# IuvenisSapiens/Qwen3-TTS-Rust

Measured on AMD Instinct MI355X. Metric: audio-seconds generated per second (aggregate over GPUs) = concurrent real-time streams; RTF and first-chunk latency from the single-utterance leg, higher is better.
Workload: dtype i8

## Files before the change

### include/q3tts.h

```cpp
#ifndef Q3TTS_H
#define Q3TTS_H
#include <stdint.h>
#include <stddef.h>
#include "q3tts_spec.h"
#ifdef __cplusplus
extern "C" {
#endif

#define Q3TTS_OK 0
#define Q3TTS_ERR -1

const char* q3tts_last_error(void);
int q3tts_version(void);
int q3tts_device_count(void);

typedef struct q3tts_sampler_config {
    float temperature;
    int32_t top_k;
    float top_p;
    int32_t has_seed;
    uint64_t seed;
} q3tts_sampler_config;
void q3tts_sampler_config_default(q3tts_sampler_config* c);

// ... 350 lines not shown
                     const int32_t* job_page0, const int32_t* job_n_pages, const int32_t* job_first, const int32_t* job_n_dst,
                     const int32_t* slots, int32_t n_slots, int32_t save);
int q3tts_op_feedback_rows(const q3tts_assets* a, const int32_t* codes, int32_t n, const int32_t* trail_ids, int32_t n_trail, float* rows);
enum { Q3TTS_GEMM_AUTO = 0, Q3TTS_GEMM_SKINNY4 = 1, Q3TTS_GEMM_SKINNY8 = 2, Q3TTS_GEMM_SKINNY16 = 3,
       Q3TTS_GEMM_F32_1 = 4, Q3TTS_GEMM_F32_2 = 5,
       Q3TTS_GEMM_H1 = 6, Q3TTS_GEMM_H1_EPL = 7, Q3TTS_GEMM_H2 = 8, Q3TTS_GEMM_H2_EPL = 9,
       Q3TTS_GEMM_H3 = 10, Q3TTS_GEMM_H3_EPL = 11 };
enum { Q3TTS_EPI_NONE = 0, Q3TTS_EPI_GELU = 1, Q3TTS_EPI_RES_SCALE = 2 , Q3TTS_EPI_RES = 3 ,
       Q3TTS_EPI_SNAKE = 4  };
typedef struct q3tts_codec_gemm_desc {
    int32_t M, N, cin, taps, dil;
    const float* A; int64_t a_rows; int32_t lda, a_segT, a_skip;
    int32_t a_split, o_split;
    const float* W; const float* bias;
    int32_t epi; const float* res; int64_t res_floats; int32_t ldr, r_segT; int64_t r_skip;
    const float* scale; const float* snake_ea; const float* snake_ib;
    float* out; int64_t out_floats, out_off; int32_t ldo, o_segT; int64_t o_skip;
    int64_t ws_floats;
    int32_t form, ksplit, reducer;
    int32_t form_ran, ksplit_ran, reducer_ran;
} q3tts_codec_gemm_desc;
int q3tts_op_codec_gemm(q3tts_codec_gemm_desc* d);
int q3tts_codec_gemm_plan(q3tts_codec_gemm_desc* d);

enum { Q3TTS_CK_RVQ_SUM = 0, Q3TTS_CK_RMSNORM_ROWS = 1, Q3TTS_CK_LAYERNORM_ROWS = 2, Q3TTS_CK_ROPE_APPEND = 3, Q3TTS_CK_WINDOW_ATTN = 4,
       Q3TTS_CK_SWIGLU_ROWS = 5, Q3TTS_CK_DWCONV7 = 6, Q3TTS_CK_SNAKE = 7, Q3TTS_CK_SNAKE_SPLIT = 8, Q3TTS_CK_CONV_OUT_WAVE = 9,
       Q3TTS_CK_CONV_OUT_WIN = 10, Q3TTS_CK_HIST_LOAD = 11, Q3TTS_CK_HIST_SAVE = 12, Q3TTS_CK_HIST_ZERO = 13 };
typedef struct q3tts_codec_kernel_desc {
    int32_t kernel;
    int32_t G, T, C, H;
    int32_t n_heads, head_dim, window; float rope_base, eps, bias;
    const int64_t* meta;
    const int64_t* codes; int32_t n_q, cb_size;
    int32_t n_streams, stream;
    const float* in[3]; int64_t in_floats[3];
    const float* p0; const float* p1; int64_t p0_floats, p1_floats;
    float* out[3]; int64_t out_floats[3];
} q3tts_codec_kernel_desc;
int q3tts_op_codec_kernel(q3tts_codec_kernel_desc* d);

enum { Q3TTS_ATTN_AUTO = 0, Q3TTS_ATTN_UNFUSED = 1 , Q3TTS_ATTN_FUSED = 2 ,
       Q3TTS_ATTN_SHORT1 = 3, Q3TTS_ATTN_SHORT2 = 4 , Q3TTS_ATTN_GGML = 5  };
typedef struct q3tts_attention_desc {
    int32_t n_head, n_kv, n_layer, layer, ntok;
    const float* qkv; int32_t qkv_stride;
    const float* q_norm; const float* k_norm;
// ... 121 lines not shown
```

### qwen3-tts-rust_amd/csrc/capi_ops.cpp

```cpp
#include "../../include/q3tts.h"
#include "transformer.h"
#include "host_logic.h"
#include "kdev.h"
#include "codec.h"
#include "kernels.h"
#include "pcm_out.h"
#include "tsm.h"
#include "mel.h"

using namespace q3;
#define Q3_API_BEGIN try {
#define Q3_API_END(failval) } catch (const std::exception& ex) { set_last_error(ex.what()); return failval; } catch (...) { set_last_error("unknown error"); return failval; }
static void require_gpu() {
    int n = 0;
    if (hipGetDeviceCount(&n) != hipSuccess || n <= 0) throw Error("no HIP device available: the HIP path is the only compute path (no CPU fallback)");
}

static int attention_op_plan(const q3tts_attention_desc& d) {
    AttnPlanIn a;
    a.ntok = d.ntok; a.fused = d.fused != 0; a.fused_max_tok = d.fused_max_tok; a.same_seq = d.same_seq != 0; a.short_attn_min = d.short_attn_min;
    a.n_head = d.n_head; a.n_kv = d.n_kv; a.hpw1_max = d.hpw1_max > 0 ? d.hpw1_max : short_attn_hpw1_max();
    a.float_mode = d.float_mode != 0; a.ggml_mode = d.ggml_mode != 0;
    return plan_attention(a);
}
// ... 859 lines not shown
        else launch_sample_pred(0, a, B);
        Q3_LAUNCH_CHECK();
    }
    Q3_HIP(hipDeviceSynchronize());
    dout.download((q3_u64*)d.out_raw, raw.size());
    ddraw.download(d.draws_out, B);
    for (int i = 0; i < nl; i++) for (int b = 0; b < B; b++) d.tokens[(size_t)i * B + b] = key_code(d.out_raw[(size_t)i * slots + (size_t)b * d.out_stride]);
    return Q3TTS_OK;
    Q3_API_END(Q3TTS_ERR)
}

int q3tts_op_codec_gemm(q3tts_codec_gemm_desc* d) {
    Q3_API_BEGIN
    require_gpu();
    codec_gemm_run(d);
    return Q3TTS_OK;
    Q3_API_END(Q3TTS_ERR)
}

int q3tts_codec_gemm_plan(q3tts_codec_gemm_desc* d) {
    Q3_API_BEGIN
    codec_gemm_plan_only(d);
    return Q3TTS_OK;
    Q3_API_END(Q3TTS_ERR)
}

int q3tts_op_codec_kernel(q3tts_codec_kernel_desc* d) {
    Q3_API_BEGIN
    require_gpu();
    codec_kernel_run(d);
    return Q3TTS_OK;
    Q3_API_END(Q3TTS_ERR)
}

int q3tts_op_project(const float* x, const float* w, const float* b, int32_t n_in, int32_t n_out, float* y) {
    Q3_API_BEGIN
    require_gpu();
    Q3_CHECK(x && w && b && y && n_in >= 1 && n_out >= 1, "bad arguments");
    const std::vector<float> wb = project_wblk(w, n_in, n_out);
    DevBuf<float> dx(n_in), dw(wb.size()), db(n_out), dy(n_out);
    dx.upload(x, n_in); dw.upload(wb.data(), wb.size()); db.upload(b, n_out);
    launch_project_blk(0, dx.p, n_in, dw.p, db.p, n_in, n_out, dy.p, n_out, 1);
    Q3_LAUNCH_CHECK();
    Q3_HIP(hipDeviceSynchronize());
    dy.download(y, n_out);
    return Q3TTS_OK;
// ... 593 lines not shown
```

### qwen3-tts-rust_amd/csrc/codec.h

```cpp
#pragma once
#include "q3_common.h"
#include <memory>
#include <string>
#include <vector>

struct q3tts_codec_gemm_desc;
struct q3tts_codec_kernel_desc;

namespace q3 {

struct CodecStateEntry { std::string name; int64_t offset; int rows, cols; };

class CodecDecoder {
public:
    std::vector<CodecStateEntry> state_layout() const;
    size_t state_floats() const;
    void state_export(int stream, float* out, size_t n_floats) const;
    void state_import(int stream, const float* in, size_t n_floats);
    CodecDecoder(const std::string& gguf_path, int n_streams, int max_frames_per_call, int n_lanes = 1, int max_group = 1);
    int max_group() const;
    int n_lanes() const;
    ~CodecDecoder();
    int samples_per_frame() const;
    void reset(int stream);
    void reset_async(hipStream_t st, int stream);
    int snapshot_async(hipStream_t st, int stream);
    void restore_async(hipStream_t st, int snapshot, int stream, const float* pcm_tail = nullptr);
    void snapshot_free(int snapshot);
    size_t snapshot_bytes() const;
    int snapshots_live() const;
    int decode(hipStream_t st, int stream, const int64_t* codes, int n_frames, bool is_last, float* pcm);
    int decode_async(hipStream_t st, int stream, const int64_t* codes, int n_frames, bool is_last, float* pcm_pinned, int lane = 0);
    int decode_group_async(hipStream_t st, int G, const int* streams, const int64_t* codes, int n_frames, float* const* pcm_pinned, int lane = 0,
                           const q3tts_pcm_format* fmt = nullptr, int64_t* n_out = nullptr, const int32_t* rate = nullptr);
    void tsm_flush_async(hipStream_t st, int stream, void* dst, int64_t* n_out, int lane = 0);
    void tsm_stats(int64_t* chunks, int64_t* frames_out, int64_t* flushes) const;
    void pcm_out_stats(int64_t* chunks_converted, int64_t* samples_out) const;
    double flops_per_frame() const;
private:
    struct Impl;
    std::unique_ptr<Impl> impl_;
};

void codec_gemm_run(q3tts_codec_gemm_desc* d);
void codec_gemm_plan_only(q3tts_codec_gemm_desc* d);
void codec_kernel_run(q3tts_codec_kernel_desc* d);

}
```

### qwen3-tts-rust_amd/csrc/codec.hip

```cpp
#include "codec.h"
#include "../../include/q3tts.h"
#include "gguf.h"
#include "kernels.h"
#include "pcm_out.h"
#include "tsm.h"
#include <atomic>
#include <cmath>
#include <cstdlib>
#include <map>

namespace q3 {

typedef float f32x16 __attribute__((ext_vector_type(16)));

enum { EPI_NONE = 0, EPI_GELU = 1, EPI_RES_SCALE = 2, EPI_RES = 3, EPI_SNAKE = 4 };

struct GemmArgs {
    const float* A; int lda;
    int cin, dil;
    const float* W;
    const float* wscale;
    const float* bias;
    float* out; int ldo;
    int M, N, K;
// ... 258 lines not shown
        for (int e = tid; e < BM * (BN / 4); e += 256) {
            const int rl = e / (BN / 4), cl = (e % (BN / 4)) * 4, row = m0 + rl, col = n0 + cl;
            if (row >= g.M || col >= g.N) continue;
            const float4 t4 = *reinterpret_cast<const float4*>(&Ct[rl][cl]);
            if (ksplit > 1) *reinterpret_cast<float4*>(g.ws + ((size_t)blockIdx.z * g.M + row) * g.N + col) = t4;
            else gemm_epilogue_store4(g, t4, row, col);
        }
    } else {
        const int col = n0 + wn * 32 + (lane & 31);
        if (col < g.N) {
#pragma unroll
            for (int t = 0; t < MR; t++)
#pragma unroll
                for (int r = 0; r < 16; r++) {
                    const int row = m0 + (wm * MR + t) * 32 + (r & 3) + 8 * (r >> 2) + 4 * (lane >> 5);
                    if (row < g.M) {
                        if (ksplit > 1) g.ws[((size_t)blockIdx.z * g.M + row) * g.N + col] = acc[t][r];
                        else gemm_store(g, row, col, gemm_epilogue(g, acc[t][r], row, col));
                    }
                }
        }
    }
}
template <int MR, int NT, int BK, int EPL, int PF, bool SPLIT>
__global__ void __launch_bounds__(256) k_conv_gemm_h3(GemmArgs g, const _Float16* __restrict__ Wh, const _Float16* __restrict__ Wl) {
    constexpr int BM = 128 * MR, BN = 32 * NT, LD = BK + 8;
    constexpr int KQ = BK / 4, KC = BK / 8;
    constexpr int NA = BM * KQ / 256;
    constexpr int NB = (BN * KC + 255) / 256;
    constexpr int CLD = BN + 4;
    struct Stage { _Float16 Ah[BM][LD], Al[BM][LD], Bh[BN][LD], Bl[BN][LD]; };
    union Shared { Stage s; float Ct[EPL ? BM : 1][CLD]; };
    __shared__ __attribute__((aligned(16))) Shared sh;
    auto& Ah = sh.s.Ah; auto& Al = sh.s.Al; auto& Bh = sh.s.Bh; auto& Bl = sh.s.Bl;
    const int tid = threadIdx.x, lane = tid & 63, wave = tid >> 6;
    int tile_m = blockIdx.y, tile_n = blockIdx.x;
    if (g.xcd_swizzle) {
        const int nwg = gridDim.x * gridDim.y, orig = blockIdx.y * gridDim.x + blockIdx.x;
        const int xcd = orig & 7, q8 = nwg >> 3, r8 = nwg & 7;
        const int wgid = (xcd < r8 ? xcd * (q8 + 1) : r8 * (q8 + 1) + (xcd - r8) * q8) + (orig >> 3);
        tile_n = wgid % gridDim.x; tile_m = wgid / gridDim.x;
    }
    const int m0 = tile_m * BM, n0 = tile_n * BN;
    const int ksplit = gridDim.z, kper = g.K / ksplit, kbeg = blockIdx.z * kper, kend = kbeg + kper;
    f32x16 acc[MR][NT];
#pragma unroll
    for (int t = 0; t < MR; t++)
#pragma unroll
        for (int u = 0; u < NT; u++)
#pragma unroll
            for (int i = 0; i < 16; i++) acc[t][u][i] = 0.0f;
    int arow[NA];
#pragma unroll
    for (int i = 0; i < NA; i++) { int mm = m0 + (tid + i * 256) / KQ; mm = mm < g.M ? mm : g.M - 1; arow[i] = mm + seg_of(mm, g.a_segT) * g.a_skip; }
    struct Regs { float4 ra[NA]; uint4 rh[NB], rl[NB]; };
    auto fetch = [&](Regs& s, int k0) {
        const int j = k0 / g.cin, ci0 = k0 % g.cin;
#pragma unroll
        for (int i = 0; i < NA; i++) {
            const int kq = (tid + i * 256) % KQ;
            const size_t row = (size_t)(arow[i] + j * g.dil);
            if constexpr (SPLIT) s.ra[i] = load_a4_split_raw(g, row, ci0 + 4 * kq);
            else s.ra[i] = *reinterpret_cast<const float4*>(g.A + row * g.lda + ci0 + 4 * kq);
        }
#pragma unroll
        for (int i = 0; i < NB; i++) {
            int e = tid + i * 256;
            e = e < BN * KC ? e : e - 256;
            const int r = e / KC, wk = 8 * (e % KC);
            s.rh[i] = *reinterpret_cast<const uint4*>(Wh + (size_t)(n0 + r) * g.K + k0 + wk);
            s.rl[i] = *reinterpret_cast<const uint4*>(Wl + (size_t)(n0 + r) * g.K + k0 + wk);
        }
    };
    auto stash = [&](const Regs& s) {
#pragma unroll
        for (int i = 0; i < NA; i++) {
            const int e = tid + i * 256, r = e / KQ, kq = e % KQ;
            if constexpr (SPLIT) {
                *reinterpret_cast<float2*>(&Ah[r][4 * kq]) = make_float2(s.ra[i].x, s.ra[i].y);
                *reinterpret_cast<float2*>(&Al[r][4 * kq]) = make_float2(s.ra[i].z, s.ra[i].w);
            } else {
                const float x[4] = {s.ra[i].x, s.ra[i].y, s.ra[i].z, s.ra[i].w};
                h4v hi, lo;
#pragma unroll
                for (int c = 0; c < 4; c++) { hi[c] = (_Float16)x[c]; lo[c] = (_Float16)(x[c] - (float)hi[c]); }
                *reinterpret_cast<h4v*>(&Ah[r][4 * kq]) = hi;
                *reinterpret_cast<h4v*>(&Al[r][4 * kq]) = lo;
            }
        }
#pragma unroll
        for (int i = 0; i < NB; i++) {
            const int e = tid + i * 256, r = e / KC, wk = 8 * (e % KC);
            if (e < BN * KC) { *reinterpret_cast<uint4*>(&Bh[r][wk]) = s.rh[i]; *reinterpret_cast<uint4*>(&Bl[r][wk]) = s.rl[i]; }
        }
    };
    auto multiply = [&]() {
#pragma unroll
        for (int kk = 0; kk < BK; kk += 16) {
            const int ko = kk + 8 * (lane >> 5);
            if constexpr (MR == 1) {
                const int ar = wave * 32 + (lane & 31);
                const h8v ah = *reinterpret_cast<const h8v*>(&Ah[ar][ko]);
                const h8v al = *reinterpret_cast<const h8v*>(&Al[ar][ko]);
#pragma unroll
                for (int u = 0; u < NT; u++) {
                    const h8v bh = *reinterpret_cast<const h8v*>(&Bh[u * 32 + (lane & 31)][ko]);
                    const h8v bl = *reinterpret_cast<const h8v*>(&Bl[u * 32 + (lane & 31)][ko]);
                    acc[0][u] = __builtin_amdgcn_mfma_f32_32x32x16_f16(al, bh, acc[0][u], 0, 0, 0);
                    acc[0][u] = __builtin_amdgcn_mfma_f32_32x32x16_f16(ah, bl, acc[0][u], 0, 0, 0);
                    acc[0][u] = __builtin_amdgcn_mfma_f32_32x32x16_f16(ah, bh, acc[0][u], 0, 0, 0);
                }
            } else {
                h8v bh[NT], bl[NT];
#pragma unroll
                for (int u = 0; u < NT; u++) {
                    bh[u] = *reinterpret_cast<const h8v*>(&Bh[u * 32 + (lane & 31)][ko]);
                    bl[u] = *reinterpret_cast<const h8v*>(&Bl[u * 32 + (lane & 31)][ko]);
                }
#pragma unroll
                for (int t = 0; t < MR; t++) {
                    const int ar = (wave * MR + t) * 32 + (lane & 31);
                    const h8v ah = *reinterpret_cast<const h8v*>(&Ah[ar][ko]);
                    const h8v al = *reinterpret_cast<const h8v*>(&Al[ar][ko]);
#pragma unroll
                    for (int u = 0; u < NT; u++) {
                        acc[t][u] = __builtin_amdgcn_mfma_f32_32x32x16_f16(al, bh[u], acc[t][u], 0, 0, 0);
                        acc[t][u] = __builtin_amdgcn_mfma_f32_32x32x16_f16(ah, bl[u], acc[t][u], 0, 0, 0);
                        acc[t][u] = __builtin_amdgcn_mfma_f32_32x32x16_f16(ah, bh[u], acc[t][u], 0, 0, 0);
                    }
                    __builtin_amdgcn_sched_barrier(0);
                }
            }
        }
    };
    auto lds_barrier = [] { asm volatile("s_waitcnt lgkmcnt(0)\n\ts_barrier" ::: "memory"); };
    float wsc[NT];
#pragma unroll
    for (int u = 0; u < NT; u++) wsc[u] = g.wscale[n0 + u * 32 + (lane & 31)];
    Regs st[PF];
#pragma unroll
    for (int j = 0; j < PF; j++)
        if (kbeg + j * BK < kend) fetch(st[j], kbeg + j * BK);
    int k0 = kbeg;
    for (; k0 + 2 * PF * BK <= kend; k0 += PF * BK) {
#pragma unroll
        for (int j = 0; j < PF; j++) {
            stash(st[j]);
            lds_barrier();
            fetch(st[j], k0 + (j + PF) * BK);
            multiply();
            lds_barrier();
        }
    }
    for (; k0 < kend; k0 += PF * BK) {
#pragma unroll
        for (int j = 0; j < PF; j++) {
            if (k0 + j * BK < kend) {
                stash(st[j]);
                lds_barrier();
                if (k0 + (j + PF) * BK < kend) fetch(st[j], k0 + (j + PF) * BK);
                multiply();
                lds_barrier();
            }
        }
    }
#pragma unroll
    for (int u = 0; u < NT; u++)
#pragma unroll
        for (int t = 0; t < MR; t++)
#pragma unroll
            for (int r = 0; r < 16; r++) acc[t][u][r] *= wsc[u];
    __syncthreads();
    auto epilogue_rows = [&](const f32x16 (&a)[NT], int row0) {
#pragma unroll
        for (int r = 0; r < 16; r++) {
            const int row = row0 + (r & 3) + 8 * (r >> 2) + 4 * (lane >> 5);
            if (row < g.M) {
#pragma unroll
                for (int u = 0; u < NT; u++) {
                    const int col = n0 + u * 32 + (lane & 31);
                    if (col < g.N) {
                        if (ksplit > 1) g.ws[((size_t)blockIdx.z * g.M + row) * g.N + col] = a[u][r];
                        else gemm_store(g, row, col, gemm_epilogue(g, a[u][r], row, col));
                    }
                }
// ... 141 lines not shown
    const bool skinny = f <= Q3TTS_GEMM_SKINNY16, f32 = f == Q3TTS_GEMM_F32_1 || f == Q3TTS_GEMM_F32_2, h3 = f >= Q3TTS_GEMM_H3;
    const bool epl = f == Q3TTS_GEMM_H1_EPL || f == Q3TTS_GEMM_H2_EPL || f == Q3TTS_GEMM_H3_EPL;
    const bool ws_a16 = (reinterpret_cast<uintptr_t>(g.ws) & 15) == 0;
    if (skinny) {
        if (g.M > (f == Q3TTS_GEMM_SKINNY4 ? 4 : f == Q3TTS_GEMM_SKINNY8 ? 8 : 16)) return "skinny form: M exceeds its row count";
        if (p.ks != 1) return "skinny form: no split-K";
        return nullptr;
    }
    if (f32 && (g.cin % 16 != 0 || (g.K / p.ks) % 16 != 0)) return "f32 form: cin and K / ksplit must be multiples of 16";
    if (!f32) {
        if (!has_split_w || !g.wscale) return "split-f16 form without split weights";
        if (g.cin % 32 != 0 || (g.K / p.ks) % 32 != 0) return "split-f16 form: cin and K / ksplit must be multiples of 32";
        if (h3 && g.N % 96 != 0) return "h3 form: N must be a multiple of 96";
        if (epl && !(epilogue4_ok(g) && ws_a16)) return "16-byte epilogue form: pointers / strides not 16-byte aligned or N % 4 != 0";
    }
    if (p.ks > 1) {
        if (p.ks > 64) return "ksplit too large";
        if ((size_t)p.ks * g.M * g.N > ws_floats) return "split-K workspace too small";
        if (p.red != 0 && p.red != 1) return "split-K needs a reducer (0 or 1)";
        if (p.red == 1 && !(epilogue4_ok(g) && ws_a16)) return "k_splitk_reduce4: pointers / strides not 16-byte aligned or N % 4 != 0";
    } else if (p.red != -1) return "a reducer without split-K";
    return nullptr;
}
static void launch_gemm(hipStream_t st, const GemmArgs& g, const GemmPlan& p, const _Float16* wh, const _Float16* wl) {
    const dim3 b256(256);
    const unsigned ks = (unsigned)p.ks;
#define Q3_H(MRV, EPLV, GRID) do { if (g.a_split) hipLaunchKernelGGL((k_conv_gemm_h<MRV, EPLV, true>), GRID, b256, 0, st, g, wh, wl); \
                                   else hipLaunchKernelGGL((k_conv_gemm_h<MRV, EPLV, false>), GRID, b256, 0, st, g, wh, wl); } while (0)
#define Q3_H3(EPLV, PFV) do { if (g.a_split) hipLaunchKernelGGL((k_conv_gemm_h3<1, 3, 32, EPLV, PFV, true>), grid3, b256, 0, st, g, wh, wl); \
                              else hipLaunchKernelGGL((k_conv_gemm_h3<1, 3, 32, EPLV, PFV, false>), grid3, b256, 0, st, g, wh, wl); } while (0)
    const dim3 grid_sk((g.N + 7) / 8), grid_t((g.N + 63) / 64, (g.M + 127) / 128, ks), grid_s((g.N + 63) / 64, (g.M + 63) / 64, ks);
    const dim3 grid3(g.N / 96, (g.M + 127) / 128, ks);
    switch (p.form) {
    case Q3TTS_GEMM_SKINNY4: hipLaunchKernelGGL((k_skinny_gemm<4>), grid_sk, dim3(512), 0, st, g); break;
    case Q3TTS_GEMM_SKINNY8: hipLaunchKernelGGL((k_skinny_gemm<8>), grid_sk, dim3(512), 0, st, g); break;
    case Q3TTS_GEMM_SKINNY16: hipLaunchKernelGGL((k_skinny_gemm<16>), grid_sk, dim3(512), 0, st, g); break;
    case Q3TTS_GEMM_F32_1: hipLaunchKernelGGL((k_conv_gemm<1>), dim3((g.N + 127) / 128, (g.M + 31) / 32, ks), b256, 0, st, g); break;
    case Q3TTS_GEMM_F32_2: hipLaunchKernelGGL((k_conv_gemm<2>), dim3((g.N + 63) / 64, (g.M + 63) / 64, ks), b256, 0, st, g); break;
    case Q3TTS_GEMM_H1: Q3_H(1, 0, grid_s); break;
    case Q3TTS_GEMM_H1_EPL: Q3_H(1, 1, grid_s); break;
    case Q3TTS_GEMM_H2: Q3_H(2, 0, grid_t); break;
    case Q3TTS_GEMM_H2_EPL: Q3_H(2, 1, grid_t); break;
    case Q3TTS_GEMM_H3: Q3_H3(0, 1); break;
    case Q3TTS_GEMM_H3_EPL: Q3_H3(1, 1); break;
    default: throw Error("unknown GEMM form");
    }
#undef Q3_H
#undef Q3_H3
    if (p.ks > 1) {
        const size_t n = (size_t)g.M * g.N;
        if (p.red == 1) hipLaunchKernelGGL(k_splitk_reduce4, dim3((unsigned)((n / 4 + 255) / 256)), b256, 0, st, g, p.ks);
        else hipLaunchKernelGGL(k_splitk_reduce, dim3((unsigned)((n + 255) / 256)), b256, 0, st, g, p.ks);
    }
}
static int xcd_swizzle_on() { static const int on = [] { const char* e = std::getenv("Q3_CODEC_XCD"); return e ? atoi(e) : 1; }(); return on; }
static void gemm(hipStream_t st, GemmArgs g, float* ws, size_t ws_floats, const _Float16* wh = nullptr, const _Float16* wl = nullptr) {
    g.ws = ws;
    g.xcd_swizzle = xcd_swizzle_on();
    launch_gemm(st, g, plan_gemm(g, ws_floats, wh != nullptr), wh, wl);
}

struct RowMap { int segT, skip, off; };
__device__ __forceinline__ size_t map_row(const RowMap& m, int r) { return (size_t)r + (size_t)(m.segT == SEG_NONE ? 0 : r / m.segT) * m.skip + m.off; }
static RowMap plain_map() { return RowMap{SEG_NONE, 0, 0}; }

__global__ void k_rvq_sum(const int64_t* __restrict__ codes, const float* const* __restrict__ cb, int n_q, int cb_size, int cb_dim,
                          float* __restrict__ out, int ldo, RowMap om) {
    const int t = blockIdx.y, d = blockIdx.x * 256 + threadIdx.x;
    if (d >= cb_dim) return;
    float acc = 0.0f;
    for (int q = 0; q < n_q; q++) {
// ... 930 lines not shown
static void check_desc(const q3tts_codec_gemm_desc& d) {
    Q3_CHECK(d.M >= 1 && d.N >= 1 && d.cin >= 1 && d.taps >= 1 && d.dil >= 1 && d.epi >= EPI_NONE && d.epi <= EPI_SNAKE, "bad codec GEMM descriptor");
    Q3_CHECK(d.a_segT >= 0 && d.o_segT >= 0 && d.r_segT >= 0 && d.a_skip >= 0 && d.o_skip >= 0 && d.r_skip >= 0 && d.out_off >= 0 && d.ws_floats >= 0,
             "negative segment / offset fields");
    Q3_CHECK(d.A && d.W && d.out && d.lda >= d.cin && d.ldo >= d.N, "codec GEMM: A, W and out are required; lda >= cin, ldo >= N");
    const long long m = d.M - 1;
    const long long arow = m + (d.a_segT > 0 ? m / d.a_segT * d.a_skip : 0) + (long long)(d.taps - 1) * d.dil;
    Q3_CHECK(arow < d.a_rows, "A rows read beyond a_rows");
    Q3_CHECK(d.out_off + m * d.ldo + (d.o_segT > 0 ? m / d.o_segT * d.o_skip : 0) + d.N <= d.out_floats, "output rows beyond out_floats");
    if (d.epi == EPI_RES || d.epi == EPI_RES_SCALE)
        Q3_CHECK(d.res && d.ldr >= d.N && m * d.ldr + (d.r_segT > 0 ? m / d.r_segT * d.r_skip : 0) + d.N <= d.res_floats, "residual rows beyond res_floats");
    Q3_CHECK(d.epi != EPI_RES_SCALE || d.scale, "EPI_RES_SCALE needs scale");
    Q3_CHECK(d.epi != EPI_SNAKE || (d.snake_ea && d.snake_ib), "EPI_SNAKE needs ea / ib");
}
void codec_gemm_plan_only(q3tts_codec_gemm_desc* d) {
    Q3_CHECK(d && d->M >= 1 && d->N >= 1 && d->cin >= 1 && d->taps >= 1 && d->out_off >= 0, "bad codec GEMM descriptor");
    GemmArgs g = desc_args(*d);
    auto at = [](const float* p, long long off) { return reinterpret_cast<float*>((p ? reinterpret_cast<uintptr_t>(p) : (uintptr_t)256) + 4 * (uintptr_t)off); };
    g.A = at(d->A, 0); g.W = at(d->W, 0); g.bias = d->bias; g.res = at(d->res, 0); g.scale = at(d->scale, 0);
    g.snake_ea = at(d->snake_ea, 0); g.snake_ib = at(d->snake_ib, 0); g.out = at(d->out, d->out_off); g.ws = at(nullptr, 0);
    const GemmPlan p = plan_gemm(g, (size_t)d->ws_floats, true);
    d->form_ran = p.form; d->ksplit_ran = p.ks; d->reducer_ran = p.red;
}
void codec_gemm_run(q3tts_codec_gemm_desc* d) {
    Q3_CHECK(d, "null codec GEMM descriptor");
    check_desc(*d);
    GemmArgs g = desc_args(*d);
    const int N = g.N, K = g.K;
    const bool res_used = g.epi == EPI_RES || g.epi == EPI_RES_SCALE;
    DevBuf<float> dA((size_t)d->a_rows * d->lda), dW((size_t)N * K), dsc(N), dbias(d->bias ? N : 0), dres(res_used ? d->res_floats : 0);
    DevBuf<float> dscale(d->scale ? N : 0), dea(d->snake_ea ? N : 0), dib(d->snake_ib ? N : 0), dout(d->out_floats), dws(std::max<int64_t>(d->ws_floats, 4));
    DevBuf<_Float16> dwh((size_t)N * K), dwl((size_t)N * K);
    g.A = dA.p; g.W = dW.p; g.wscale = dsc.p; g.bias = dbias.p; g.res = dres.p; g.scale = dscale.p; g.snake_ea = dea.p; g.snake_ib = dib.p;
    g.out = dout.p + d->out_off; g.ws = dws.p;
    const GemmPlan p = d->form == Q3TTS_GEMM_AUTO ? plan_gemm(g, (size_t)d->ws_floats, true) : GemmPlan{d->form, d->ksplit, d->reducer};
    if (const char* why = gemm_plan_error(g, p, (size_t)d->ws_floats, true)) throw Error(std::string("codec GEMM form not applicable: ") + why);
    std::vector<_Float16> h((size_t)N * K), l((size_t)N * K);
    std::vector<float> sc(N);
    split_weights(d->W, N, K, h.data(), l.data(), sc.data());
    dA.upload(d->A, dA.n); dW.upload(d->W, dW.n); dwh.upload(h.data(), h.size()); dwl.upload(l.data(), l.size()); dsc.upload(sc.data(), N);
    if (d->bias) dbias.upload(d->bias, N);
    if (res_used) dres.upload(d->res, dres.n);
    if (d->scale) dscale.upload(d->scale, N);
    if (d->snake_ea) dea.upload(d->snake_ea, N);
    if (d->snake_ib) dib.upload(d->snake_ib, N);
    dout.upload(d->out, dout.n);
// ... 112 lines not shown
```

### qwen3-tts-rust_amd/python/q3tts/__init__.py

```python
import ctypes as C
import os
import numpy as np

_HERE = os.path.dirname(os.path.abspath(__file__))
PKG_ROOT = os.path.dirname(os.path.dirname(_HERE))
LIB_PATH = os.path.join(PKG_ROOT, "libq3tts.so")
_lib = None


class Q3Error(RuntimeError):
    pass


class SamplerConfig(C.Structure):
    _fields_ = [("temperature", C.c_float), ("top_k", C.c_int32), ("top_p", C.c_float), ("has_seed", C.c_int32),
                ("seed", C.c_uint64)]


class GenOptions(C.Structure):
    _fields_ = [("repetition_penalty", C.c_float), ("predictor_temperature", C.c_float), ("predictor_top_k", C.c_int32),
                ("predictor_top_p", C.c_float)]


GEN_DEFAULTS = {"repetition_penalty": 1.0, "predictor_temperature": 0.0, "predictor_top_k": 0, "predictor_top_p": 1.0}
# ... 34 lines not shown
    "q3tts_engine_create", "q3tts_engine_destroy", "q3tts_generate_batch", "q3tts_engine_stats", "q3tts_engine_reset_stats",
    "q3tts_engine_set_instrument", "q3tts_engine_bytes_per_step", "q3tts_assets_open", "q3tts_assets_close", "q3tts_engine_assets",
    "q3tts_assets_codec_embedding", "q3tts_assets_text_embedding", "q3tts_assets_tts_pad", "q3tts_prompt_build_core",
    "q3tts_prompt_build_clone", "q3tts_sampler_new", "q3tts_sampler_free", "q3tts_sampler_sample", "q3tts_chunker_new",
    "q3tts_chunker_free", "q3tts_chunker_push", "q3tts_decoder_create", "q3tts_decoder_destroy", "q3tts_decoder_samples_per_frame",
    "q3tts_decoder_reset", "q3tts_decoder_decode", "q3tts_mel_frames", "q3tts_mel", "q3tts_tf_open", "q3tts_tf_close",
    "q3tts_tf_dims", "q3tts_tf_clear", "q3tts_tf_eval", "q3tts_op_gemv_q8", "q3tts_op_gateup_q8", "q3tts_op_matmul_float", "q3tts_op_rmsnorm_quant", "q3tts_op_swiglu_quant",
    "q3tts_op_argmax", "q3tts_op_project", "q3tts_op_sample", "q3tts_submit", "q3tts_poll", "q3tts_fetch", "q3tts_wait",
    "q3tts_release", "q3tts_decoder_create_ex", "q3tts_decoder_decode_group", "q3tts_sched_start", "q3tts_sched_stop", "q3tts_sched_step", "q3tts_voice_register", "q3tts_submit_text",
    "q3tts_group_create", "q3tts_group_destroy", "q3tts_group_size", "q3tts_group_engine", "q3tts_group_uses_rccl", "q3tts_group_voice_register",
    "q3tts_group_submit", "q3tts_group_submit_text", "q3tts_group_device_of", "q3tts_group_poll", "q3tts_group_fetch", "q3tts_group_wait",
    "q3tts_group_release", "q3tts_group_start", "q3tts_group_stop", "q3tts_comm_available", "q3tts_comm_unique_id", "q3tts_comm_create",
    "q3tts_comm_destroy", "q3tts_comm_voice_register", "q3tts_engine_device",
    "q3tts_onnx_open", "q3tts_onnx_close", "q3tts_onnx_counts", "q3tts_onnx_summary", "q3tts_onnx_node", "q3tts_onnx_node_input", "q3tts_onnx_node_output",
    "q3tts_onnx_node_attr_ints", "q3tts_onnx_node_attr_float", "q3tts_onnx_initializer", "q3tts_onnx_op_kernel", "q3tts_onnx_decoder_contract",
    "q3tts_onnx_session_open", "q3tts_onnx_session_close", "q3tts_onnx_session_unsupported", "q3tts_onnx_session_set_input", "q3tts_onnx_session_run",
    "q3tts_onnx_session_output_info", "q3tts_onnx_session_output", "q3tts_onnx_session_launches", "q3tts_onnx_op_executable",
    "q3tts_text_nfc", "q3tts_op_gemv_kq", "q3tts_op_gateup_kq", "q3tts_onnx_decoder_open", "q3tts_onnx_decoder_close", "q3tts_onnx_decoder_reset", "q3tts_onnx_decoder_fetch", "q3tts_group_info", "q3tts_onnx_decoder_decode",
    "q3tts_decoder_state_floats", "q3tts_decoder_state_export", "q3tts_decoder_state_import", "q3tts_decoder_state_entry",
    "q3tts_tokenizer_open", "q3tts_tokenizer_close", "q3tts_tokenizer_encode", "q3tts_tokenizer_decode", "q3tts_tokenizer_vocab_size",
    "q3tts_gen_options_default", "q3tts_submit_ex", "q3tts_submit_text_ex", "q3tts_generate_batch_ex", "q3tts_group_submit_ex",
    "q3tts_group_submit_text_ex", "q3tts_op_sample_rows",
    "q3tts_prompt_build_streaming", "q3tts_submit_trailing", "q3tts_submit_text_streaming", "q3tts_generate_batch_trailing",
    "q3tts_group_submit_text_streaming", "q3tts_op_codec_gemm", "q3tts_codec_gemm_plan", "q3tts_op_codec_kernel", "q3tts_op_attention", "q3tts_attention_plan",
    "q3tts_op_linear", "q3tts_linear_plan", "q3tts_argmax_key",
    "q3tts_submit_trailing_open", "q3tts_trail_append", "q3tts_trail_progress", "q3tts_submit_text_streaming_open", "q3tts_text_append",
    "q3tts_group_submit_text_streaming_open", "q3tts_group_text_append", "q3tts_group_trail_append", "q3tts_group_trail_progress",
    "q3tts_cancel", "q3tts_group_cancel",
    "q3tts_submit_resume", "q3tts_group_submit_resume", "q3tts_op_feedback_rows", "q3tts_engine_prefill_width",
    "q3tts_engine_set_logprobs", "q3tts_fetch_logprobs", "q3tts_group_set_logprobs", "q3tts_group_fetch_logprobs", "q3tts_op_logprob_rows",
    "q3tts_submit_score", "q3tts_group_submit_score", "q3tts_engine_score_width", "q3tts_op_score_rows", "q3tts_op_score_inputs",
    "q3tts_pred_table_bytes", "q3tts_op_attention_keyed", "q3tts_op_select_rows", "q3tts_op_frame_glue", "q3tts_op_ggml",
    "q3tts_submit_candidates", "q3tts_group_submit_candidates", "q3tts_engine_candidate_stats", "q3tts_op_kv_fork",
    "q3tts_submit_decode", "q3tts_group_submit_decode", "q3tts_engine_decode_width", "q3tts_engine_decode_stats",
    "q3tts_engine_set_output_format", "q3tts_request_format", "q3tts_fetch_pcm16", "q3tts_engine_pcm_out_stats",
    "q3tts_group_set_output_format", "q3tts_group_fetch_pcm16", "q3tts_group_request_format",
    "q3tts_pcm_out_plan", "q3tts_pcm_out_filter", "q3tts_pcm_out_samples", "q3tts_pcm_format_check", "q3tts_op_pcm_convert",
    "q3tts_decoder_snapshot_create", "q3tts_decoder_snapshot_restore", "q3tts_decoder_snapshot_free", "q3tts_decoder_snapshot_bytes",
    "q3tts_preamble_create", "q3tts_preamble_poll", "q3tts_preamble_wait", "q3tts_preamble_release", "q3tts_voice_set_preamble",
    "q3tts_engine_set_preamble", "q3tts_request_preamble", "q3tts_engine_preamble_stats",
    "q3tts_group_preamble_create", "q3tts_group_preamble_wait", "q3tts_group_preamble_release", "q3tts_group_voice_set_preamble",
    "q3tts_group_set_preamble", "q3tts_group_request_preamble",
    "q3tts_stem_create", "q3tts_voice_stem_create", "q3tts_stem_poll", "q3tts_stem_wait", "q3tts_stem_release", "q3tts_voice_set_stem",
    "q3tts_engine_set_stem", "q3tts_request_stem", "q3tts_engine_stem_stats", "q3tts_op_kv_stem",
    "q3tts_group_stem_create", "q3tts_group_voice_stem_create", "q3tts_group_stem_wait", "q3tts_group_stem_release",
    "q3tts_group_voice_set_stem", "q3tts_group_set_stem", "q3tts_group_request_stem", "q3tts_group_stem_stats",
    "q3tts_engine_set_speech_rate", "q3tts_request_speech_rate", "q3tts_engine_tsm_stats", "q3tts_group_set_speech_rate",
# ... 1238 lines not shown
    assert out.dtype.itemsize == 4
    vecs = [None if v is None else np.ascontiguousarray(v, np.float32) for v in (bias, scale, ea, ib)]
    for v in vecs:
        assert v is None or v.size == N
    res = None if res is None else np.ascontiguousarray(res, np.float32).reshape(-1)
    d = _codec_gemm_desc(M, N, cin, taps, dil, A.shape[1], A.shape[0], a_segT, a_skip, epi, ldr, 0 if res is None else res.size, r_segT, r_skip,
                         ldo, out.size, out_off, o_segT, o_skip, a_split, o_split, ws_floats, form, ksplit, reducer)
    d.A, d.W, d.out, d.res = _p(A), _p(W), _p(out), _p(res)
    d.bias, d.scale, d.snake_ea, d.snake_ib = (_p(v) for v in vecs)
    lib().q3tts_op_codec_gemm.argtypes = [C.POINTER(CodecGemmDesc)]
    _chk(lib().q3tts_op_codec_gemm(C.byref(d)))
    return out, (GEMM_FORM_NAMES[d.form_ran], d.ksplit_ran, d.reducer_ran)


def codec_gemm_plan(M, N, cin, taps=1, dil=1, lda=None, ldo=None, out_off=0, o_segT=0, o_skip=0, a_segT=0, a_skip=0, epi=EPI_NONE, ldr=0,
                    r_segT=0, r_skip=0, a_split=False, o_split=False, ws_floats=1 << 22):
    d = _codec_gemm_desc(M, N, cin, taps, dil, cin if lda is None else lda, 0, a_segT, a_skip, epi, ldr, 0, r_segT, r_skip,
                         N if ldo is None else ldo, 0, out_off, o_segT, o_skip, a_split, o_split, ws_floats, 0, 1, -1)
    lib().q3tts_codec_gemm_plan.argtypes = [C.POINTER(CodecGemmDesc)]
    _chk(lib().q3tts_codec_gemm_plan(C.byref(d)))
    return GEMM_FORM_NAMES[d.form_ran], d.ksplit_ran, d.reducer_ran


CODEC_KERNELS = {"RVQ_SUM": 0, "RMSNORM_ROWS": 1, "LAYERNORM_ROWS": 2, "ROPE_APPEND": 3, "WINDOW_ATTN": 4, "SWIGLU_ROWS": 5, "DWCONV7": 6,
                 "SNAKE": 7, "SNAKE_SPLIT": 8, "CONV_OUT_WAVE": 9, "CONV_OUT_WIN": 10, "HIST_LOAD": 11, "HIST_SAVE": 12, "HIST_ZERO": 13}
CODEC_MAX_FRAMES = 65536


class CodecKernelDesc(C.Structure):
    _fields_ = [("kernel", C.c_int32), ("G", C.c_int32), ("T", C.c_int32), ("C", C.c_int32), ("H", C.c_int32),
                ("n_heads", C.c_int32), ("head_dim", C.c_int32), ("window", C.c_int32), ("rope_base", C.c_float), ("eps", C.c_float),
                ("bias", C.c_float), ("meta", C.c_void_p), ("codes", C.c_void_p), ("n_q", C.c_int32), ("cb_size", C.c_int32),
                ("n_streams", C.c_int32), ("stream", C.c_int32), ("inp", C.c_void_p * 3), ("in_floats", C.c_int64 * 3),
                ("p0", C.c_void_p), ("p1", C.c_void_p), ("p0_floats", C.c_int64), ("p1_floats", C.c_int64),
                ("out", C.c_void_p * 3), ("out_floats", C.c_int64 * 3)]


def op_codec_kernel(kernel, G, T, C_, H=0, ins=(), outs=(), p0=None, p1=None, meta=None, codes=None, n_q=0, cb_size=0, n_heads=0,
                    head_dim=0, window=0, rope_base=10000.0, eps=1e-5, bias=0.0, n_streams=0, stream=0):
    d = CodecKernelDesc()
    d.kernel = CODEC_KERNELS[kernel] if isinstance(kernel, str) else kernel
    d.G, d.T, d.C, d.H = G, T, C_, H
    d.n_heads, d.head_dim, d.window, d.rope_base, d.eps, d.bias = n_heads, head_dim, window, rope_base, eps, bias
    d.n_q, d.cb_size, d.n_streams, d.stream = n_q, cb_size, n_streams, stream
    keep = []
    if meta is not None:
# ... 728 lines not shown
```

Measured before the change: 741.0.

## Reuse staged activation halo across conv taps in H3 codec GEMM

```diff
diff --git a/include/q3tts.h b/include/q3tts.h
--- a/include/q3tts.h
+++ b/include/q3tts.h
@@ -396,6 +396,7 @@
 } q3tts_codec_gemm_desc;
 int q3tts_op_codec_gemm(q3tts_codec_gemm_desc* d);
 int q3tts_codec_gemm_plan(q3tts_codec_gemm_desc* d);
+int q3tts_codec_gemm_tap_reuse(const q3tts_codec_gemm_desc* d);
 
 enum { Q3TTS_CK_RVQ_SUM = 0, Q3TTS_CK_RMSNORM_ROWS = 1, Q3TTS_CK_LAYERNORM_ROWS = 2, Q3TTS_CK_ROPE_APPEND = 3, Q3TTS_CK_WINDOW_ATTN = 4,
        Q3TTS_CK_SWIGLU_ROWS = 5, Q3TTS_CK_DWCONV7 = 6, Q3TTS_CK_SNAKE = 7, Q3TTS_CK_SNAKE_SPLIT = 8, Q3TTS_CK_CONV_OUT_WAVE = 9,
diff --git a/qwen3-tts-rust_amd/csrc/capi_ops.cpp b/qwen3-tts-rust_amd/csrc/capi_ops.cpp
--- a/qwen3-tts-rust_amd/csrc/capi_ops.cpp
+++ b/qwen3-tts-rust_amd/csrc/capi_ops.cpp
@@ -905,6 +905,12 @@
     Q3_API_BEGIN
     codec_gemm_plan_only(d);
     return Q3TTS_OK;
+    Q3_API_END(Q3TTS_ERR)
+}
+
+int q3tts_codec_gemm_tap_reuse(const q3tts_codec_gemm_desc* d) {
+    Q3_API_BEGIN
+    return codec_gemm_tap_reuse(d);
     Q3_API_END(Q3TTS_ERR)
 }
 
diff --git a/qwen3-tts-rust_amd/csrc/codec.h b/qwen3-tts-rust_amd/csrc/codec.h
--- a/qwen3-tts-rust_amd/csrc/codec.h
+++ b/qwen3-tts-rust_amd/csrc/codec.h
@@ -44,6 +44,7 @@
 
 void codec_gemm_run(q3tts_codec_gemm_desc* d);
 void codec_gemm_plan_only(q3tts_codec_gemm_desc* d);
+int codec_gemm_tap_reuse(const q3tts_codec_gemm_desc* d);
 void codec_kernel_run(q3tts_codec_kernel_desc* d);
 
 }
diff --git a/qwen3-tts-rust_amd/csrc/codec.hip b/qwen3-tts-rust_amd/csrc/codec.hip
--- a/qwen3-tts-rust_amd/csrc/codec.hip
+++ b/qwen3-tts-rust_amd/csrc/codec.hip
@@ -304,14 +304,18 @@
         }
     }
 }
-template <int MR, int NT, int BK, int EPL, int PF, bool SPLIT>
-__global__ void __launch_bounds__(256) k_conv_gemm_h3(GemmArgs g, const _Float16* __restrict__ Wh, const _Float16* __restrict__ Wl) {
+constexpr int H3_HALO_ROWS = 240;
+template <int MR, int NT, int BK, int EPL, int PF, bool SPLIT, bool TAPS = false>
+__global__ void __launch_bounds__(256) __attribute__((amdgpu_waves_per_eu(TAPS ? 3 : 1))) k_conv_gemm_h3(GemmArgs g, const _Float16* __restrict__ Wh, const _Float16* __restrict__ Wl) {
     constexpr int BM = 128 * MR, BN = 32 * NT, LD = BK + 8;
     constexpr int KQ = BK / 4, KC = BK / 8;
     constexpr int NA = BM * KQ / 256;
     constexpr int NB = (BN * KC + 255) / 256;
     constexpr int CLD = BN + 4;
-    struct Stage { _Float16 Ah[BM][LD], Al[BM][LD], Bh[BN][LD], Bl[BN][LD]; };
+    constexpr int AR = TAPS ? H3_HALO_ROWS : BM;
+    constexpr int NH = (AR * KQ + 255) / 256;
+    static_assert(!TAPS || (MR == 1 && PF == 1), "the tap-reusing loop is written for the 128-row tile, one K tile in flight");
+    struct Stage { _Float16 Ah[AR][LD], Al[AR][LD], Bh[BN][LD], Bl[BN][LD]; };
     union Shared { Stage s; float Ct[EPL ? BM : 1][CLD]; };
     __shared__ __attribute__((aligned(16))) Shared sh;
     auto& Ah = sh.s.Ah; auto& Al = sh.s.Al; auto& Bh = sh.s.Bh; auto& Bl = sh.s.Bl;
@@ -335,55 +339,60 @@
     int arow[NA];
 #pragma unroll
     for (int i = 0; i < NA; i++) { int mm = m0 + (tid + i * 256) / KQ; mm = mm < g.M ? mm : g.M - 1; arow[i] = mm + seg_of(mm, g.a_segT) * g.a_skip; }
-    struct Regs { float4 ra[NA]; uint4 rh[NB], rl[NB]; };
-    auto fetch = [&](Regs& s, int k0) {
-        const int j = k0 / g.cin, ci0 = k0 % g.cin;
-#pragma unroll
-        for (int i = 0; i < NA; i++) {
-            const int kq = (tid + i * 256) % KQ;
-            const size_t row = (size_t)(arow[i] + j * g.dil);
-            if constexpr (SPLIT) s.ra[i] = load_a4_split_raw(g, row, ci0 + 4 * kq);
-            else s.ra[i] = *reinterpret_cast<const float4*>(g.A + row * g.lda + ci0 + 4 * kq);
-        }
+    typedef unsigned u4v __attribute__((ext_vector_type(4)));
+    struct Regs { float4 ra[NA]; u4v rh[NB], rl[NB]; };
+    auto load_a = [&](size_t row, int ci) {
+        if constexpr (SPLIT) return load_a4_split_raw(g, row, ci);
+        else return *reinterpret_cast<const float4*>(g.A + row * g.lda + ci);
+    };
+    auto split_store = [&](const float4& v, int r, int c) {
+        if constexpr (SPLIT) {
+            *reinterpret_cast<float2*>(&Ah[r][c]) = make_float2(v.x, v.y);
+            *reinterpret_cast<float2*>(&Al[r][c]) = make_float2(v.z, v.w);
+        } else {
+            const float x[4] = {v.x, v.y, v.z, v.w};
+            h4v hi, lo;
+#pragma unroll
+            for (int c4 = 0; c4 < 4; c4++) { hi[c4] = (_Float16)x[c4]; lo[c4] = (_Float16)(x[c4] - (float)hi[c4]); }
+            *reinterpret_cast<h4v*>(&Ah[r][c]) = hi;
+            *reinterpret_cast<h4v*>(&Al[r][c]) = lo;
+        }
+    };
+    auto fetch_b = [&](u4v (&rh)[NB], u4v (&rl)[NB], int k0) {
 #pragma unroll
         for (int i = 0; i < NB; i++) {
             int e = tid + i * 256;
             e = e < BN * KC ? e : e - 256;
             const int r = e / KC, wk = 8 * (e % KC);
-            s.rh[i] = *reinterpret_cast<const uint4*>(Wh + (size_t)(n0 + r) * g.K + k0 + wk);
-            s.rl[i] = *reinterpret_cast<const uint4*>(Wl + (size_t)(n0 + r) * g.K + k0 + wk);
+            rh[i] = *reinterpret_cast<const u4v*>(Wh + (size_t)(n0 + r) * g.K + k0 + wk);
+            rl[i] = *reinterpret_cast<const u4v*>(Wl + (size_t)(n0 + r) * g.K + k0 + wk);
+        }
+    };
+    auto fetch = [&](Regs& s, int k0) {
+        const int j = k0 / g.cin, ci0 = k0 % g.cin;
+#pragma unroll
+        for (int i = 0; i < NA; i++) s.ra[i] = load_a((size_t)(arow[i] + j * g.dil), ci0 + 4 * ((tid + i * 256) % KQ));
+        fetch_b(s.rh, s.rl, k0);
+    };
+    auto stash_b = [&](const u4v (&rh)[NB], const u4v (&rl)[NB]) {
+#pragma unroll
+        for (int i = 0; i < NB; i++) {
+            const int e = tid + i * 256, r = e / KC, wk = 8 * (e % KC);
+            if (e < BN * KC) { *reinterpret_cast<u4v*>(&Bh[r][wk]) = rh[i]; *reinterpret_cast<u4v*>(&Bl[r][wk]) = rl[i]; }
         }
     };
     auto stash = [&](const Regs& s) {
 #pragma unroll
-        for (int i = 0; i < NA; i++) {
-            const int e = tid + i * 256, r = e / KQ, kq = e % KQ;
-            if constexpr (SPLIT) {
-                *reinterpret_cast<float2*>(&Ah[r][4 * kq]) = make_float2(s.ra[i].x, s.ra[i].y);
-                *reinterpret_cast<float2*>(&Al[r][4 * kq]) = make_float2(s.ra[i].z, s.ra[i].w);
-            } else {
-                const float x[4] = {s.ra[i].x, s.ra[i].y, s.ra[i].z, s.ra[i].w};
-                h4v hi, lo;
-#pragma unroll
-                for (int c = 0; c < 4; c++) { hi[c] = (_Float16)x[c]; lo[c] = (_Float16)(x[c] - (float)hi[c]); }
-                *reinterpret_cast<h4v*>(&Ah[r][4 * kq]) = hi;
-                *reinterpret_cast<h4v*>(&Al[r][4 * kq]) = lo;
-            }
-        }
-#pragma unroll
-        for (int i = 0; i < NB; i++) {
-            const int e = tid + i * 256, r = e / KC, wk = 8 * (e % KC);
-            if (e < BN * KC) { *reinterpret_cast<uint4*>(&Bh[r][wk]) = s.rh[i]; *reinterpret_cast<uint4*>(&Bl[r][wk]) = s.rl[i]; }
-        }
+        for (int i = 0; i < NA; i++) { const int e = tid + i * 256; split_store(s.ra[i], e / KQ, 4 * (e % KQ)); }
+        stash_b(s.rh, s.rl);
     };
-    auto multiply = [&]() {
+    auto multiply = [&](int ar0) {
 #pragma unroll
         for (int kk = 0; kk < BK; kk += 16) {
             const int ko = kk + 8 * (lane >> 5);
             if constexpr (MR == 1) {
-                const int ar = wave * 32 + (lane & 31);
-                const h8v ah = *reinterpret_cast<const h8v*>(&Ah[ar][ko]);
-                const h8v al = *reinterpret_cast<const h8v*>(&Al[ar][ko]);
+                const h8v ah = *reinterpret_cast<const h8v*>(&Ah[ar0][ko]);
+                const h8v al = *reinterpret_cast<const h8v*>(&Al[ar0][ko]);
 #pragma unroll
                 for (int u = 0; u < NT; u++) {
                     const h8v bh = *reinterpret_cast<const h8v*>(&Bh[u * 32 + (lane & 31)][ko]);
@@ -419,30 +428,70 @@
     float wsc[NT];
 #pragma unroll
     for (int u = 0; u < NT; u++) wsc[u] = g.wscale[n0 + u * 32 + (lane & 31)];
-    Regs st[PF];
-#pragma unroll
-    for (int j = 0; j < PF; j++)
-        if (kbeg + j * BK < kend) fetch(st[j], kbeg + j * BK);
-    int k0 = kbeg;
-    for (; k0 + 2 * PF * BK <= kend; k0 += PF * BK) {
-#pragma unroll
-        for (int j = 0; j < PF; j++) {
-            stash(st[j]);
+    if constexpr (TAPS) {
+        const int taps = g.K / g.cin, nchunk = g.cin / BK;
+        const int mlast = (m0 + BM < g.M ? m0 + BM : g.M) - 1;
+        const int p0 = m0 + seg_of(m0, g.a_segT) * g.a_skip;
+        const int span = mlast + seg_of(mlast, g.a_segT) * g.a_skip + (taps - 1) * g.dil - p0 + 1;
+        int mm = m0 + wave * 32 + (lane & 31); mm = mm < g.M ? mm : g.M - 1;
+        const int aoff = mm + seg_of(mm, g.a_segT) * g.a_skip - p0;
+        const int hr0 = tid / KQ, hc = 4 * (tid % KQ);
+        float4 ha[NH];
+        u4v wh[NB], wl[NB];
+        auto fetch_halo = [&](int ci0) {
+#pragma unroll
+            for (int i = 0; i < NH; i++) { const int r = hr0 + i * (256 / KQ); ha[i] = load_a((size_t)(p0 + (r < span ? r : span - 1)), ci0 + hc); }
+        };
+        auto stash_halo = [&] {
+#pragma unroll
+            for (int i = 0; i < NH; i++) { const int r = hr0 + i * (256 / KQ); if (r < span) split_store(ha[i], r, hc); }
+        };
+        fetch_halo(0);
+        fetch_b(wh, wl, 0);
+        for (int c = 0; c < nchunk; c++) {
+            const int ci0 = c * BK, cnext = (c + 1 < nchunk ? c + 1 : c) * BK;
+            stash_halo();
+            stash_b(wh, wl);
             lds_barrier();
-            fetch(st[j], k0 + (j + PF) * BK);
-            multiply();
+            fetch_halo(cnext);
+            fetch_b(wh, wl, g.cin + ci0);
+            multiply(aoff);
             lds_barrier();
-        }
-    }
-    for (; k0 < kend; k0 += PF * BK) {
-#pragma unroll
-        for (int j = 0; j < PF; j++) {
-            if (k0 + j * BK < kend) {
+            for (int j = 1; j < taps; j++) {
+                stash_b(wh, wl);
+                lds_barrier();
+                fetch_b(wh, wl, j + 1 < taps ? (j + 1) * g.cin + ci0 : cnext);
+                multiply(aoff + j * g.dil);
+                lds_barrier();
+            }
+        }
+    } else {
+        const int ar0 = wave * 32 + (lane & 31);
+        Regs st[PF];
+#pragma unroll
+        for (int j = 0; j < PF; j++)
+            if (kbeg + j * BK < kend) fetch(st[j], kbeg + j * BK);
+        int k0 = kbeg;
+        for (; k0 + 2 * PF * BK <= kend; k0 += PF * BK) {
+#pragma unroll
+            for (int j = 0; j < PF; j++) {
                 stash(st[j]);
                 lds_barrier();
-                if (k0 + (j + PF) * BK < kend) fetch(st[j], k0 + (j + PF) * BK);
-                multiply();
+                fetch(st[j], k0 + (j + PF) * BK);
+                multiply(ar0);
                 lds_barrier();
+            }
+        }
+        for (; k0 < kend; k0 += PF * BK) {
+#pragma unroll
+            for (int j = 0; j < PF; j++) {
+                if (k0 + j * BK < kend) {
+                    stash(st[j]);
+                    lds_barrier();
+                    if (k0 + (j + PF) * BK < kend) fetch(st[j], k0 + (j + PF) * BK);
+                    multiply(ar0);
+                    lds_barrier();
+                }
             }
         }
     }
@@ -630,13 +679,33 @@
     } else if (p.red != -1) return "a reducer without split-K";
     return nullptr;
 }
+static int h3_halo_span(const GemmArgs& g) {
+    const int taps = g.K / g.cin, ntiles = (g.M + 127) / 128;
+    int period = 1;
+    if (g.a_segT != SEG_NONE) { int a = g.a_segT, b = 128; while (b) { const int t = a % b; a = b; b = t; } period = g.a_segT / a; }
+    const bool whole = ntiles > period;
+    int span = 0;
+    for (int t = 0; t < (whole ? period : ntiles); t++) {
+        const int m0 = t * 128, m1 = (whole || m0 + 128 < g.M ? m0 + 128 : g.M) - 1;
+        const int s0 = g.a_segT == SEG_NONE ? 0 : m0 / g.a_segT, s1 = g.a_segT == SEG_NONE ? 0 : m1 / g.a_segT;
+        span = std::max(span, m1 - m0 + (s1 - s0) * g.a_skip + (taps - 1) * g.dil + 1);
+    }
+    return span;
+}
+static bool h3_tap_reuse(const GemmArgs& g, const GemmPlan& p) {
+    static const int on = [] { const char* e = std::getenv("Q3_CODEC_H3_TAPS"); return e ? atoi(e) : 1; }();
+    if (!on || (p.form != Q3TTS_GEMM_H3 && p.form != Q3TTS_GEMM_H3_EPL) || p.ks != 1 || g.cin % 32 != 0 || g.K / g.cin < 2) return false;
+    return h3_halo_span(g) <= H3_HALO_ROWS;
+}
 static void launch_gemm(hipStream_t st, const GemmArgs& g, const GemmPlan& p, const _Float16* wh, const _Float16* wl) {
     const dim3 b256(256);
     const unsigned ks = (unsigned)p.ks;
+    const bool taps = h3_tap_reuse(g, p);
 #define Q3_H(MRV, EPLV, GRID) do { if (g.a_split) hipLaunchKernelGGL((k_conv_gemm_h<MRV, EPLV, true>), GRID, b256, 0, st, g, wh, wl); \
                                    else hipLaunchKernelGGL((k_conv_gemm_h<MRV, EPLV, false>), GRID, b256, 0, st, g, wh, wl); } while (0)
-#define Q3_H3(EPLV, PFV) do { if (g.a_split) hipLaunchKernelGGL((k_conv_gemm_h3<1, 3, 32, EPLV, PFV, true>), grid3, b256, 0, st, g, wh, wl); \
-                              else hipLaunchKernelGGL((k_conv_gemm_h3<1, 3, 32, EPLV, PFV, false>), grid3, b256, 0, st, g, wh, wl); } while (0)
+#define Q3_H3T(EPLV, PFV, TAPSV) do { if (g.a_split) hipLaunchKernelGGL((k_conv_gemm_h3<1, 3, 32, EPLV, PFV, true, TAPSV>), grid3, b256, 0, st, g, wh, wl); \
+                                      else hipLaunchKernelGGL((k_conv_gemm_h3<1, 3, 32, EPLV, PFV, false, TAPSV>), grid3, b256, 0, st, g, wh, wl); } while (0)
+#define Q3_H3(EPLV, PFV) do { if (taps) Q3_H3T(EPLV, PFV, true); else Q3_H3T(EPLV, PFV, false); } while (0)
     const dim3 grid_sk((g.N + 7) / 8), grid_t((g.N + 63) / 64, (g.M + 127) / 128, ks), grid_s((g.N + 63) / 64, (g.M + 63) / 64, ks);
     const dim3 grid3(g.N / 96, (g.M + 127) / 128, ks);
     switch (p.form) {
@@ -655,6 +724,7 @@
     }
 #undef Q3_H
 #undef Q3_H3
+#undef Q3_H3T
     if (p.ks > 1) {
         const size_t n = (size_t)g.M * g.N;
         if (p.red == 1) hipLaunchKernelGGL(k_splitk_reduce4, dim3((unsigned)((n / 4 + 255) / 256)), b256, 0, st, g, p.ks);
@@ -1631,6 +1701,13 @@
     const GemmPlan p = plan_gemm(g, (size_t)d->ws_floats, true);
     d->form_ran = p.form; d->ksplit_ran = p.ks; d->reducer_ran = p.red;
 }
+int codec_gemm_tap_reuse(const q3tts_codec_gemm_desc* d) {
+    Q3_CHECK(d && d->M >= 1 && d->N >= 1 && d->cin >= 1 && d->taps >= 1 && d->dil >= 1 && d->out_off >= 0, "bad codec GEMM descriptor");
+    q3tts_codec_gemm_desc c = *d;
+    if (c.form == Q3TTS_GEMM_AUTO) codec_gemm_plan_only(&c);
+    else { c.form_ran = c.form; c.ksplit_ran = c.ksplit; c.reducer_ran = c.reducer; }
+    return h3_tap_reuse(desc_args(*d), GemmPlan{c.form_ran, c.ksplit_ran, c.reducer_ran}) ? 1 : 0;
+}
 void codec_gemm_run(q3tts_codec_gemm_desc* d) {
     Q3_CHECK(d, "null codec GEMM descriptor");
     check_desc(*d);
diff --git a/qwen3-tts-rust_amd/python/q3tts/__init__.py b/qwen3-tts-rust_amd/python/q3tts/__init__.py
--- a/qwen3-tts-rust_amd/python/q3tts/__init__.py
+++ b/qwen3-tts-rust_amd/python/q3tts/__init__.py
@@ -80,7 +80,7 @@
     "q3tts_gen_options_default", "q3tts_submit_ex", "q3tts_submit_text_ex", "q3tts_generate_batch_ex", "q3tts_group_submit_ex",
     "q3tts_group_submit_text_ex", "q3tts_op_sample_rows",
     "q3tts_prompt_build_streaming", "q3tts_submit_trailing", "q3tts_submit_text_streaming", "q3tts_generate_batch_trailing",
-    "q3tts_group_submit_text_streaming", "q3tts_op_codec_gemm", "q3tts_codec_gemm_plan", "q3tts_op_codec_kernel", "q3tts_op_attention", "q3tts_attention_plan",
+    "q3tts_group_submit_text_streaming", "q3tts_op_codec_gemm", "q3tts_codec_gemm_plan", "q3tts_codec_gemm_tap_reuse", "q3tts_op_codec_kernel", "q3tts_op_attention", "q3tts_attention_plan",
     "q3tts_op_linear", "q3tts_linear_plan", "q3tts_argmax_key",
     "q3tts_submit_trailing_open", "q3tts_trail_append", "q3tts_trail_progress", "q3tts_submit_text_streaming_open", "q3tts_text_append",
     "q3tts_group_submit_text_streaming_open", "q3tts_group_text_append", "q3tts_group_trail_append", "q3tts_group_trail_progress",
@@ -1365,6 +1365,17 @@
     return GEMM_FORM_NAMES[d.form_ran], d.ksplit_ran, d.reducer_ran
 
 
+def codec_gemm_tap_reuse(M, N, cin, taps=1, dil=1, lda=None, ldo=None, out_off=0, o_segT=0, o_skip=0, a_segT=0, a_skip=0, epi=EPI_NONE, ldr=0,
+                         r_segT=0, r_skip=0, a_split=False, o_split=False, ws_floats=1 << 22, form="AUTO", ksplit=1, reducer=-1):
+    d = _codec_gemm_desc(M, N, cin, taps, dil, cin if lda is None else lda, 0, a_segT, a_skip, epi, ldr, 0, r_segT, r_skip,
+                         N if ldo is None else ldo, 0, out_off, o_segT, o_skip, a_split, o_split, ws_floats, form, ksplit, reducer)
+    lib().q3tts_codec_gemm_tap_reuse.argtypes = [C.POINTER(CodecGemmDesc)]
+    r = lib().q3tts_codec_gemm_tap_reuse(C.byref(d))
+    if r < 0:
+        _chk(r)
+    return bool(r)
+
+
 CODEC_KERNELS = {"RVQ_SUM": 0, "RMSNORM_ROWS": 1, "LAYERNORM_ROWS": 2, "ROPE_APPEND": 3, "WINDOW_ATTN": 4, "SWIGLU_ROWS": 5, "DWCONV7": 6,
                  "SNAKE": 7, "SNAKE_SPLIT": 8, "CONV_OUT_WAVE": 9, "CONV_OUT_WIN": 10, "HIST_LOAD": 11, "HIST_SAVE": 12, "HIST_ZERO": 13}
 CODEC_MAX_FRAMES = 65536
```

New measurement: 757.5 (median of 6 runs). 1.02x the previous value.
